# Layjins/Spider

Measured on AMD Instinct MI355X. Metric: multimodal responses/sec (text->text+image), higher is better.
Workload: dtype bf16

## Files before the change

### include/spider_hip.h

```cpp
#ifndef SPIDER_HIP_H
#define SPIDER_HIP_H
#define SPIDER_ABI_VERSION 4

#ifdef __cplusplus
extern "C" {
#endif

int spider_abi_version(void);
const char* spider_target_arch(void);
const char* spider_last_error(void);


int spider_embed_bf16(const void* table, const int* ids, void* out, int rows, int H, int V, void* stream);

int spider_rmsnorm_bf16(const void* x, const void* res, const void* w, void* y, void* res_out, int rows, int H,
                        float eps, void* stream);

int spider_gemv_bf16(const void* W, const void* x, void* out, const void* bias, const void* res, const void* norm_w,
                     float eps, int B, int N, int K, void* stream);

int spider_gemv_swiglu_bf16(const void* W_gate_up, const void* x, void* out, const void* norm_w, float eps, int B,
                            int I, int K, void* stream);

int spider_lm_head_nparts(int V);
// ... 22 lines not shown
int spider_sample_partial_bf16(const void* logits, const void* seen, const void* ban, const float* penalty, const int* min_new,
                               const int* eos_ids, const int* n_eos, const int* n_hist, const int* top_k, float* ws_val,
                               int* ws_tok, int rows, int V, int nslice, void* stream);
int spider_sample_select_f32(const float* ws_val, const int* ws_tok, const float* temperature, const float* top_p, const int* top_k,
                             const void* seed, const int* row0, const int* n_hist, int* next_ids, int* cand_tok, float* cand_p,
                             int* n_keep, float* u, int rows, int V, int nslice, void* stream);

int spider_rope_kv_append_bf16(const void* qkv, const int* pos, const int* slot, const float* cos_sin, void* q_out,
                               void* k_cache, void* v_cache, int B, int S, int n_q, int n_kv, int d, int T_max,
                               void* stream);
int spider_rope_kv_append_mrope_bf16(const void* qkv, const int* pos3, const int* slot, const float* cos_sin, void* q_out,
                                     void* k_cache, void* v_cache, int B, int S, int n_q, int n_kv, int d, int T_max,
                                     int sec_t, int sec_h, void* stream);

int spider_attn_decode_bf16(const void* q, const void* k_cache, const void* v_cache, const int* kv_beg,
                            const int* kv_end, void* out, void* ws_o, void* ws_ml, int B, int n_q, int n_kv, int d,
                            int T_max, float scale, int nsplit, void* stream);

int spider_attn_decode_fused_bf16(const void* qkv, const int* pos, const float* cos_sin, void* k_cache, void* v_cache,
                                  const int* kv_beg, const int* kv_end, void* out, void* ws_o, void* ws_ml,
                                  int* counters, int B, int n_q, int n_kv, int d, int T_max, float scale, int nsplit,
                                  void* stream);
int spider_set_attn_inline(int on);
int spider_set_gemv_sched(int sched);
int spider_set_ws_inlaunch(int on);

int spider_gemv_fm_bf16(const void* Wfm, const void* x, void* out, const void* bias, const void* res, int B, int N, int K,
                        int fold_rmsnorm, float eps, void* stream);
int spider_gemv_swiglu_fm_bf16(const void* Wfm_gate_up, const void* x, void* out, int B, int I, int K, int fold_rmsnorm, float eps,
                               void* stream);
int spider_lm_head_argmax_fm_bf16(const void* Wfm, const void* x, int* out_ids, void* logits, void* ws_val, void* ws_idx, int B,
                                  int V, int K, int fold_rmsnorm, float eps, void* stream);
int spider_lm_head_argmax_fm_proc_bf16(const void* Wfm, const void* x, int* out_ids, void* logits, void* ws_val, void* ws_idx,
                                       const void* seen, const void* ban, const float* penalty, const int* min_new,
                                       const int* eos_ids, const int* n_eos, const int* n_hist, int B, int V, int K,
                                       int fold_rmsnorm, float eps, void* stream);


int spider_gemm_bf16(const void* A, const void* W, void* C, void* C32, const void* bias, const void* res,
                     const void* rowbias, int rows_per_group, int M, int N, int K, int lda, int ldc, int act,
                     float out_scale, int w_tiled, const float* res32, float* c32d, void* ws, long ws_bytes, void* stream);

int spider_gemm_ln_bf16(const void* A, const void* Wf, void* C, const float* colsum, const float* colbias, const void* res,
                        int M, int N, int K, int ldc, int act, float eps, int w_tiled, void* ws, long ws_bytes, void* stream);

int spider_xattn_fused_bf16(const void* x, const void* mq_fm, const void* mo_fm, const float* colsum, const float* colbias,
// ... 193 lines not shown
```

### spider_amd/csrc/llm_decode.hip

```cpp
#include "common.hpp"
#include "select.hpp"
#include <stdlib.h>

using namespace spider;

__global__ __launch_bounds__(256) void embed_kernel(const bf16_t* __restrict__ table, const int* __restrict__ ids,
                                                    bf16_t* __restrict__ out, int H, int V) {
    const int r = blockIdx.x;
    int id = ids[r];
    id = id < 0 ? 0 : (id >= V ? V - 1 : id);
    const u32x4* src = reinterpret_cast<const u32x4*>(table + (size_t)id * H);
    u32x4* dst = reinterpret_cast<u32x4*>(out + (size_t)r * H);
    for (int i = threadIdx.x; i < H / 8; i += 256) dst[i] = src[i];
}

__global__ __launch_bounds__(256) void rope_rows_kernel(bf16_t* __restrict__ x, const float* __restrict__ cs, long row_stride,
                                                        int rows, int heads, int d) {
    const int half = d >> 1, cpr = half >> 3;
    const long total = (long)rows * heads * cpr;
    for (long idx = (long)blockIdx.x * 256 + threadIdx.x; idx < total; idx += (long)gridDim.x * 256) {
        const int c = (int)(idx % cpr);
        const int h = (int)((idx / cpr) % heads);
        const long r = idx / ((long)cpr * heads);
        bf16_t* p = x + r * row_stride + (long)h * d + c * 8;
// ... 803 lines not shown
            o0 = o0 * a + ovv[u].x * bsc;
            o1 = o1 * a + ovv[u].y * bsc;
            m = mn;
        }
    }
    if (lane == 0) { sm_m[wave] = m; sm_l[wave] = l; }
    sm_o[wave][lane * 2] = o0;
    sm_o[wave][lane * 2 + 1] = o1;
    __syncthreads();
    if (threadIdx.x < D) {
        const int dd = threadIdx.x;
        float mm = fmaxf(fmaxf(sm_m[0], sm_m[1]), fmaxf(sm_m[2], sm_m[3]));
        float ll = 0.f, oo = 0.f;
#pragma unroll
        for (int w = 0; w < 4; ++w) {
            const float a = (sm_m[w] == -INFINITY) ? 0.f : __expf(sm_m[w] - mm);
            ll += sm_l[w] * a;
            oo += sm_o[w][dd] * a;
        }
        out[bh * D + dd] = f32_to_bf16(ll > 0.f ? oo / ll : 0.f);
    }
}

template <int D, int G, int NWV, int UR>
__global__ __launch_bounds__(NWV * 64) void attn_decode_fused_kernel(
    const bf16_t* __restrict__ qkv, const int* __restrict__ pos, const float* __restrict__ cs, bf16_t* __restrict__ kc,
    bf16_t* __restrict__ vc, const int* __restrict__ kv_beg, const int* __restrict__ kv_end, float* __restrict__ part_o,
    float* __restrict__ part_ml, int* __restrict__ cnt, bf16_t* __restrict__ out, int n_kv, int T_max, float scale,
    int nsplit, int inline_combine) {
    static_assert(D == 128, "decode attention is specialised for head_dim 128");
    constexpr int HALF = D / 2;
    const int split = blockIdx.x, hk = blockIdx.y, b = blockIdx.z;
    const int n_q = n_kv * G;
    const int lane = threadIdx.x & 63, wave = threadIdx.x >> 6;
    const int sub = lane >> 4;
    const int dl = (lane & 15) * 8;
    const bool hi_half = dl >= HALF;
    const int dp = hi_half ? dl - HALF : dl + HALF;
    const int beg = kv_beg ? kv_beg[b] : 0, end = kv_end[b];
    const int t_new = end - 1;
    const int len_old = max(t_new - beg, 0);
    const int per = (len_old + nsplit - 1) / nsplit;
    const int t0 = beg + split * per, t1 = min(t_new, t0 + per);

    const bf16_t* kbase = kc + ((size_t)b * n_kv + hk) * (size_t)T_max * D;
    const bf16_t* vbase = vc + ((size_t)b * n_kv + hk) * (size_t)T_max * D;
    constexpr int RSTEP = 4 * NWV;
    auto load_rows = [&](int tb_, u32x4 (&kr)[UR], u32x4 (&vr)[UR]) {
#pragma unroll
        for (int u = 0; u < UR; ++u) {
            const int t = min(tb_ + RSTEP * u, t1 - 1);
            kr[u] = *reinterpret_cast<const u32x4*>(kbase + (size_t)t * D + dl);
            vr[u] = *reinterpret_cast<const u32x4*>(vbase + (size_t)t * D + dl);
        }
    };
    const int tb0 = t0 + wave * 4 + sub;
// ... 6 lines not shown
    {
        const int ci = hi_half ? dl - HALF : dl;
        const f32x4 c0 = *reinterpret_cast<const f32x4*>(c + ci), c1 = *reinterpret_cast<const f32x4*>(c + ci + 4);
        const f32x4 s0 = *reinterpret_cast<const f32x4*>(c + HALF + ci), s1 = *reinterpret_cast<const f32x4*>(c + HALF + ci + 4);
#pragma unroll
        for (int j = 0; j < 4; ++j) { cosv[j] = c0[j]; cosv[4 + j] = c1[j]; sinv[j] = s0[j]; sinv[4 + j] = s1[j]; }
    }
    auto rope8 = [&](const bf16_t* head, float (&o)[8]) {
        const u32x4 a = *reinterpret_cast<const u32x4*>(head + dl), pq = *reinterpret_cast<const u32x4*>(head + dp);
        const uint32_t aw[4] = {a.x, a.y, a.z, a.w}, pw[4] = {pq.x, pq.y, pq.z, pq.w};
#pragma unroll
        for (int j = 0; j < 8; ++j) {
            const float xv = (j & 1) ? bf16hi_to_f32(aw[j >> 1]) : bf16lo_to_f32(aw[j >> 1]);
            const float pv = (j & 1) ? bf16hi_to_f32(pw[j >> 1]) : bf16lo_to_f32(pw[j >> 1]);
            const float t1_ = bf16_to_f32(f32_to_bf16(xv * cosv[j]));
            const float t2_ = bf16_to_f32(f32_to_bf16((hi_half ? pv : -pv) * sinv[j]));
            o[j] = bf16_to_f32(f32_to_bf16(t1_ + t2_));
        }
    };

    float qf[G][8];
#pragma unroll
    for (int g = 0; g < G; ++g) {
        rope8(row + (size_t)(hk * G + g) * D, qf[g]);
#pragma unroll
        for (int j = 0; j < 8; ++j) qf[g][j] *= scale;
    }
    float m[G], l[G], o[G][8];
#pragma unroll
    for (int g = 0; g < G; ++g) {
        m[g] = -INFINITY;
        l[g] = 0.f;
#pragma unroll
        for (int j = 0; j < 8; ++j) o[g][j] = 0.f;
    }
    auto update = [&](const float (&kf)[8], const float (&vf)[8]) {
#pragma unroll
        for (int g = 0; g < G; ++g) {
            float sc = 0.f;
#pragma unroll
            for (int j = 0; j < 8; ++j) sc += qf[g][j] * kf[j];
            sc += __shfl_xor(sc, 1, 64);
            sc += __shfl_xor(sc, 2, 64);
            sc += __shfl_xor(sc, 4, 64);
            sc += __shfl_xor(sc, 8, 64);
            const float mn = fmaxf(m[g], sc);
            const float alpha = __expf(m[g] - mn);
// ... 15 lines not shown
                float kf[8], vf[8];
#pragma unroll
                for (int j = 0; j < 4; ++j) {
                    kf[2 * j] = bf16lo_to_f32(kw[j]); kf[2 * j + 1] = bf16hi_to_f32(kw[j]);
                    vf[2 * j] = bf16lo_to_f32(vw[j]); vf[2 * j + 1] = bf16hi_to_f32(vw[j]);
                }
                update(kf, vf);
            }
            if (more) {
                const int t = min(tb + CHUNK + RSTEP * u, t1 - 1);
                kq[u] = *reinterpret_cast<const u32x4*>(kbase + (size_t)t * D + dl);
                vq[u] = *reinterpret_cast<const u32x4*>(vbase + (size_t)t * D + dl);
            }
        }
    }
    if (split == nsplit - 1 && wave == 0 && sub == 0 && t_new >= beg) {
        float kf[8], vf[8];
        rope8(row + (size_t)(n_q + hk) * D, kf);
        const u32x4 vq = *reinterpret_cast<const u32x4*>(row + (size_t)(n_q + n_kv + hk) * D + dl);
        const uint32_t vw[4] = {vq.x, vq.y, vq.z, vq.w};
#pragma unroll
        for (int j = 0; j < 4; ++j) { vf[2 * j] = bf16lo_to_f32(vw[j]); vf[2 * j + 1] = bf16hi_to_f32(vw[j]); }
        update(kf, vf);
        u32x4 ko;
        ko.x = pack_bf16x2(kf[0], kf[1]); ko.y = pack_bf16x2(kf[2], kf[3]);
        ko.z = pack_bf16x2(kf[4], kf[5]); ko.w = pack_bf16x2(kf[6], kf[7]);
        *reinterpret_cast<u32x4*>(kc + (((size_t)b * n_kv + hk) * T_max + t_new) * D + dl) = ko;
        *reinterpret_cast<u32x4*>(vc + (((size_t)b * n_kv + hk) * T_max + t_new) * D + dl) = vq;
    }

    __shared__ float sm_m[NWV][G], sm_l[NWV][G];
    __shared__ float sm_o[NWV][G][D];
    __shared__ int sm_last;
#pragma unroll
    for (int g = 0; g < G; ++g) {
#pragma unroll
        for (int off = 16; off <= 32; off <<= 1) {
            const float m2 = __shfl_xor(m[g], off, 64);
            const float l2 = __shfl_xor(l[g], off, 64);
            const float mn = fmaxf(m[g], m2);
            const float a1 = (m[g] == -INFINITY) ? 0.f : __expf(m[g] - mn);
            const float a2 = (m2 == -INFINITY) ? 0.f : __expf(m2 - mn);
            l[g] = l[g] * a1 + l2 * a2;
#pragma unroll
            for (int j = 0; j < 8; ++j) {
                const float o2 = __shfl_xor(o[g][j], off, 64);
                o[g][j] = o[g][j] * a1 + o2 * a2;
            }
            m[g] = mn;
        }
        if (lane < 16) {
#pragma unroll
            for (int j = 0; j < 8; ++j) sm_o[wave][g][dl + j] = o[g][j];
            if (lane == 0) { sm_m[wave][g] = m[g]; sm_l[wave][g] = l[g]; }
        }
    }
    __syncthreads();
    if (nsplit > 1 && inline_combine) {
        for (int idx = threadIdx.x; idx < G * (D / 4); idx += NWV * 64) {
            const int g = idx / (D / 4), d4 = (idx % (D / 4)) * 4;
            float mm = -INFINITY;
#pragma unroll
            for (int w = 0; w < NWV; ++w) mm = fmaxf(mm, sm_m[w][g]);
            float ll = 0.f;
            f32x4 oo = {0.f, 0.f, 0.f, 0.f};
#pragma unroll
            for (int w = 0; w < NWV; ++w) {
                const float a = (sm_m[w][g] == -INFINITY) ? 0.f : __expf(sm_m[w][g] - mm);
                ll += sm_l[w][g] * a;
#pragma unroll
                for (int j = 0; j < 4; ++j) oo[j] += sm_o[w][g][d4 + j] * a;
            }
            const size_t pi = ((size_t)b * n_q + hk * G + g) * nsplit + split;
            float* po = part_o + pi * D + d4;
            asm volatile("global_store_dwordx4 %0, %1, off sc1" ::"v"(po), "v"(oo) : "memory");
            if (d4 == 0) {
                const float2 mlv = float2{mm, ll};
                float* pm = part_ml + pi * 2;
                asm volatile("global_store_dwordx2 %0, %1, off sc1" ::"v"(pm), "v"(mlv) : "memory");
            }
        }
// ... 49 lines not shown
                }
            }
            const float inv = lsum > 0.f ? 1.f / lsum : 0.f;
            u32x2 o2;
            o2.x = pack_bf16x2(acc[0] * inv, acc[1] * inv);
            o2.y = pack_bf16x2(acc[2] * inv, acc[3] * inv);
            *reinterpret_cast<u32x2*>(out + bh * D + d4) = o2;
        }
        if (threadIdx.x == 0) __hip_atomic_store(cnt + (size_t)b * n_kv + hk, 0, __ATOMIC_RELAXED, __HIP_MEMORY_SCOPE_AGENT);
        return;
    }
    for (int idx = threadIdx.x; idx < G * D; idx += NWV * 64) {
        const int g = idx / D, dd = idx % D;
        float mm = -INFINITY;
#pragma unroll
        for (int w = 0; w < NWV; ++w) mm = fmaxf(mm, sm_m[w][g]);
        float ll = 0.f, oo = 0.f;
#pragma unroll
        for (int w = 0; w < NWV; ++w) {
            const float a = (sm_m[w][g] == -INFINITY) ? 0.f : __expf(sm_m[w][g] - mm);
            ll += sm_l[w][g] * a;
            oo += sm_o[w][g][dd] * a;
        }
        const int hq = hk * G + g;
        if (nsplit == 1) {
            out[((size_t)b * n_q + hq) * D + dd] = f32_to_bf16(ll > 0.f ? oo / ll : 0.f);
        } else {
            const size_t pi = ((size_t)b * n_q + hq) * nsplit + split;
            part_o[pi * D + dd] = oo;
            if (dd == 0) { part_ml[pi * 2] = mm; part_ml[pi * 2 + 1] = ll; }
        }
    }
}

template <bool GATEUP, int NW>
__global__ __launch_bounds__(NW * 64) void skinny_gemm_kernel(const bf16_t* __restrict__ W, const bf16_t* __restrict__ x,
                                                          bf16_t* __restrict__ out, const bf16_t* __restrict__ bias,
                                                          const bf16_t* __restrict__ res, int B, int N, int K) {
    constexpr int TN = GATEUP ? 2 : 1;
    __shared__ float part[NW][TN][64][4];
    const int lane = threadIdx.x & 63, wave = threadIdx.x >> 6;
    const int r16 = lane & 15, g = lane >> 4;
    const int n0 = blockIdx.x * 16;
    const int nrow = min(n0 + r16, N - 1);
    const bf16_t* wrow[TN];
    wrow[0] = W + (size_t)nrow * K + 16 * g;
    if (GATEUP) wrow[1] = W + (size_t)(N + nrow) * K + 16 * g;
    const bool x_ok = r16 < B;
    const bf16_t* xrow = x + (size_t)(x_ok ? r16 : 0) * K + 16 * g;

    const int nkb = K / 64;
    const int kb0 = (wave * nkb) / NW, kb1 = ((wave + 1) * nkb) / NW;
    f32x4 acc[TN];
// ... 291 lines not shown
    if (B >= mfma_min_b && B <= 16 && K % 64 == 0 && norm_w == nullptr) {
        skinny_gemm_kernel<GU, 8><<<(N + 15) / 16, 512, 0, (hipStream_t)stream>>>((const bf16_t*)W, (const bf16_t*)x, (bf16_t*)out,
                                                                                  (const bf16_t*)bias, (const bf16_t*)res, B, N, K);
        SPIDER_LAUNCH_OK();
        return 0;
    }
    switch (B) {
        case 1: return gemv_dispatch<1, GU>(W, x, out, bias, res, norm_w, eps, N, K, stream);
        case 2: return gemv_dispatch<2, GU>(W, x, out, bias, res, norm_w, eps, N, K, stream);
        case 3: return gemv_dispatch<3, GU>(W, x, out, bias, res, norm_w, eps, N, K, stream);
        case 4: return gemv_dispatch<4, GU>(W, x, out, bias, res, norm_w, eps, N, K, stream);
        case 5: return gemv_dispatch<5, GU>(W, x, out, bias, res, norm_w, eps, N, K, stream);
        case 6: return gemv_dispatch<6, GU>(W, x, out, bias, res, norm_w, eps, N, K, stream);
        case 7: return gemv_dispatch<7, GU>(W, x, out, bias, res, norm_w, eps, N, K, stream);
        case 8: return gemv_dispatch<8, GU>(W, x, out, bias, res, norm_w, eps, N, K, stream);
        default: spider_set_error("gemv: batch must be 1..8 (1..16 when K % 64 == 0 and norm_w == NULL; use spider_gemm_bf16 beyond that)"); return -1;
    }
}


#define SPIDER_ATTN_INLINE_DEFAULT 0
static int g_attn_inline = -1;

extern "C" {

int spider_set_gemv_sched(int sched) {
    const int prev = gemv_sched();
    g_gemv_sched = sched != 0;
    return prev;
}

int spider_set_attn_inline(int on) {
    const int prev = g_attn_inline;
    g_attn_inline = on < 0 ? 0 : (on > 2 ? 2 : on);
    return prev;
}

int spider_embed_bf16(const void* table, const int* ids, void* out, int rows, int H, int V, void* stream) {
    SPIDER_CHECK(rows > 0 && H > 0 && H % 8 == 0 && V > 0, "embed: bad shape (H must be a multiple of 8)");
    embed_kernel<<<rows, 256, 0, (hipStream_t)stream>>>((const bf16_t*)table, ids, (bf16_t*)out, H, V);
    SPIDER_LAUNCH_OK();
    return 0;
}

int spider_rope_rows_bf16(void* x, const float* cos_sin, long row_stride, int rows, int heads, int d, void* stream) {
    SPIDER_CHECK(rows > 0 && heads > 0 && d > 0 && d % 16 == 0, "rope_rows: head_dim must be a multiple of 16");
    SPIDER_CHECK(row_stride % 8 == 0 && row_stride >= (long)heads * d, "rope_rows: row stride must be >= heads*d and keep 16-byte alignment");
    const long total = (long)rows * heads * (d / 16);
    long g = (total + 255) / 256;
    if (g > 8192) g = 8192;
    rope_rows_kernel<<<(int)g, 256, 0, (hipStream_t)stream>>>((bf16_t*)x, cos_sin, row_stride, rows, heads, d);
    SPIDER_LAUNCH_OK();
    return 0;
}

int spider_rmsnorm_bf16(const void* x, const void* res, const void* w, void* y, void* res_out, int rows, int H,
                        float eps, void* stream) {
// ... 259 lines not shown
    const int inline_combine = g_attn_inline;
    static const int wide_env = [] { const char* e = getenv("SPIDER_ATTN_WIDE"); return e ? atoi(e) : -1; }();
    const bool wide = wide_env >= 0 ? wide_env != 0 : (T_max / nsplit >= 96);
    switch (G) {
        case 1: ATTN_FUSED_LAUNCH(1); break;
        case 2: ATTN_FUSED_LAUNCH(2); break;
        case 3: ATTN_FUSED_LAUNCH(3); break;
        case 4: ATTN_FUSED_LAUNCH(4); break;
        case 5: ATTN_FUSED_LAUNCH(5); break;
        case 6: ATTN_FUSED_LAUNCH(6); break;
        case 7: ATTN_FUSED_LAUNCH(7); break;
        case 8: ATTN_FUSED_LAUNCH(8); break;
        default: spider_set_error("attn_decode_fused: GQA group size must be 1 ... 8"); return -1;
    }
    SPIDER_LAUNCH_OK();
    if (nsplit > 1 && !inline_combine) {
        attn_combine_kernel<128><<<B * n_q, 256, 0, (hipStream_t)stream>>>((const float*)ws_o, (const float*)ws_ml,
                                                                          (bf16_t*)out, nsplit);
        SPIDER_LAUNCH_OK();
    }
    return 0;
}

}
```

### spider_amd/lib.py

```python
from __future__ import annotations

import ctypes as C
import os
import threading

import torch

_HERE = os.path.dirname(os.path.abspath(__file__))
LIB_PATH = os.path.join(_HERE, "libspider_hip.so")

_lib = None
_lock = threading.Lock()

_vp, _i, _f, _l = C.c_void_p, C.c_int, C.c_float, C.c_long

SIGNATURES = {
    "spider_abi_version": (_i, []),
    "spider_target_arch": (C.c_char_p, []),
    "spider_last_error": (C.c_char_p, []),
    "spider_embed_bf16": (_i, [_vp, _vp, _vp, _i, _i, _i, _vp]),
    "spider_rmsnorm_bf16": (_i, [_vp, _vp, _vp, _vp, _vp, _i, _i, _f, _vp]),
    "spider_gemv_bf16": (_i, [_vp, _vp, _vp, _vp, _vp, _vp, _f, _i, _i, _i, _vp]),
    "spider_gemv_swiglu_bf16": (_i, [_vp, _vp, _vp, _vp, _f, _i, _i, _i, _vp]),
    "spider_lm_head_nparts": (_i, [_i]),
    "spider_decode_advance_i32": (_i, [_vp] * 7 + [_i, _i, _vp]),
    "spider_lm_head_argmax_bf16": (_i, [_vp, _vp, _vp, _f, _vp, _vp, _vp, _vp, _i, _i, _i, _vp]),
    "spider_lm_head_argmax_proc_bf16": (_i, [_vp, _vp, _vp, _f] + [_vp] * 11 + [_i, _i, _i, _vp]),
    "spider_decode_advance_seen_i32": (_i, [_vp] * 8 + [_i, _i, _i, _vp]),
    "spider_token_bitmap_set_i32": (_i, [_vp, _vp, _i, _i, _i, _vp]),
    "spider_beam_partial_bf16": (_i, [_vp] * 4 + [_i] * 4 + [_vp]),
    "spider_beam_select_f32": (_i, [_vp] * 10 + [_i, _vp, _vp] + [_i] * 5 + [_vp]),
    "spider_kv_row_gather_bf16": (_i, [_vp] * 7 + [_i] * 7 + [_vp]),
    "spider_sample_partial_bf16": (_i, [_vp] * 11 + [_i] * 3 + [_vp]),
    "spider_sample_select_f32": (_i, [_vp] * 13 + [_i] * 3 + [_vp]),
    "spider_gemv_fm_bf16": (_i, [_vp, _vp, _vp, _vp, _vp, _i, _i, _i, _i, _f, _vp]),
    "spider_gemv_swiglu_fm_bf16": (_i, [_vp, _vp, _vp, _i, _i, _i, _i, _f, _vp]),
    "spider_lm_head_argmax_fm_bf16": (_i, [_vp, _vp, _vp, _vp, _vp, _vp, _i, _i, _i, _i, _f, _vp]),
    "spider_lm_head_argmax_fm_proc_bf16": (_i, [_vp] * 13 + [_i, _i, _i, _i, _f, _vp]),
    "spider_rope_kv_append_bf16": (_i, [_vp, _vp, _vp, _vp, _vp, _vp, _vp, _i, _i, _i, _i, _i, _i, _vp]),
    "spider_rope_kv_append_mrope_bf16": (_i, [_vp, _vp, _vp, _vp, _vp, _vp, _vp, _i, _i, _i, _i, _i, _i, _i, _i, _vp]),
    "spider_attn_decode_bf16": (_i, [_vp, _vp, _vp, _vp, _vp, _vp, _vp, _vp, _i, _i, _i, _i, _i, _f, _i, _vp]),
    "spider_attn_decode_fused_bf16": (_i, [_vp] * 11 + [_i, _i, _i, _i, _i, _f, _i, _vp]),
    "spider_set_attn_inline": (_i, [_i]),
    "spider_set_gemv_sched": (_i, [_i]),
    "spider_set_ws_inlaunch": (_i, [_i]),
    "spider_gemm_bf16": (_i, [_vp, _vp, _vp, _vp, _vp, _vp, _vp, _i, _i, _i, _i, _i, _i, _i, _f, _i, _vp, _vp, _vp, _l, _vp]),
    "spider_gemm_ln_bf16": (_i, [_vp, _vp, _vp, _vp, _vp, _vp, _i, _i, _i, _i, _i, _f, _i, _vp, _l, _vp]),
    "spider_xattn_fused_bf16": (_i, [_vp, _vp, _vp, _vp, _vp, _vp, _vp, _i, _i, _i, _i, _i, _f, _vp, _vp, _vp]),
    "spider_conv2d_nhwc_bf16": (_i, [_vp, _vp, _vp, _vp, _vp, _vp, _i, _i, _i, _i, _i, _i, _i, _i, _i, _f, _i, _vp, _vp, _vp, _l, _vp]),
    "spider_conv_nhwc_ex_bf16": (_i, [_vp] * 6 + [_i] * 14 + [_f, _f, _i, _vp, _vp, _vp, _l, _vp]),
    "spider_attn_bf16": (_i, [_vp, _vp, _vp, _vp] + [_l] * 12 + [_i] * 6 + [_f, _i, _i, _vp, _vp, _i, _i, _vp]),
    "spider_story_key_lists_i32": (_i, [_vp, _i, _i, _i, _i, _i, _i, _vp, _vp, _vp]),
    "spider_attn_keylist_bf16": (_i, [_vp, _vp, _vp, _vp] + [_l] * 12 + [_i] * 6 + [_f, _vp, _i, _vp, _i, _vp]),
    "spider_attn_varlen_bf16": (_i, [_vp, _vp, _vp, _vp, _l, _l, _l, _l, _i, _i, _i, _i, _f, _vp, _i, _vp]),
    "spider_rope_rows_bf16": (_i, [_vp, _vp, _l, _i, _i, _i, _vp]),
    "spider_groupnorm_nchunk": (_i, [_i]),
    "spider_groupnorm_nhwc_bf16": (_i, [_vp, _vp, _vp, _vp, _vp, _i, _i, _i, _i, _f, _i, _vp]),
    "spider_groupnorm_cat_nhwc_bf16": (_i, [_vp] * 7 + [_i, _i, _i, _i, _i, _f, _i, _vp]),
    "spider_conv_nhwc_gn_bf16": (_i, [_vp] * 6 + [_i] * 14 + [_f, _f, _i, _vp, _vp, _vp, _l, _vp] + [_vp, _i, _vp]),
    "spider_groupnorm_stats_nhwc_bf16": (_i, [_vp, _vp, _i, _i, _i, _i, _i, _vp]),
    "spider_groupnorm_apply_nhwc_bf16": (_i, [_vp, _vp, _i, _vp, _vp, _vp, _i, _i, _i, _i, _f, _i, _vp]),
    "spider_gemm_gn_in_bf16": (_i, [_vp, _vp, _vp, _vp, _i, _i, _i, _i, _i, _vp, _i, _vp, _vp, _i, _f, _i, _vp, _vp]),
    "spider_layernorm_bf16": (_i, [_vp, _vp, _vp, _vp, _i, _i, _f, _vp]),
    "spider_geglu_bf16": (_i, [_vp, _vp, _i, _i, _vp]),
    "spider_swiglu_bf16": (_i, [_vp, _vp, _i, _i, _vp]),
    "spider_concat_channels_bf16": (_i, [_vp, _vp, _vp, _l, _i, _i, _vp]),
# ... 78 lines not shown
```

### spider_amd/llm.py

```python
from __future__ import annotations

import os
import math
from dataclasses import dataclass
from typing import Callable, List, Optional, Sequence

import torch

from . import ops
from .graphs import capture as capture_graph

BF16 = torch.bfloat16


@dataclass
class LLMConfig:
    hidden: int
    layers: int
    n_q: int
    n_kv: int
    head_dim: int
    inter: int
    vocab: int
    rope_theta: float = 10000.0
# ... 525 lines not shown
            q = torch.empty(B, S, c.n_q, c.head_dim, dtype=BF16, device=self.device)
            ops.rope_kv_append(qkv, pos, slot, self.cos_sin, q, k_cache[l], v_cache[l], B, S, c.n_q, c.n_kv, c.head_dim,
                               mrope_section=sec)
            a = ops.attention_cache(q, k_cache[l], v_cache[l], Lk=S, causal=True, kv_off=0, kv_beg=kv_beg)
            h = ops.gemm(a.view(B * S, -1), lw["w_o"], res=h)
            x = ops.rmsnorm(h, lw["ln2"], c.eps)
            if _FUSE_SWIGLU:
                act = ops.gemm(x, lw["w_gu"], act="swiglu")
            else:
                act = ops.swiglu(ops.gemm(x, lw["w_gu"]))
            h = ops.gemm(act, lw["w_down"], res=h)
            if hidden_out is not None:
                hidden_out.append(h.view(B, S, -1).clone())
        return h

    def _decode_step(self, st: dict):
        c, B = self.cfg, st["B"]
        k_cache, v_cache = st["kv"]
        h = ops.embed(self.embed_w, st["cur_ids"]) if st["embeds_in"] is None else st["embeds_in"]
        hs = st.get("hidden_buf")
        if hs is not None:
            hs[0].copy_(h)
        fm = self.fm_batch and B >= self.FM_MIN_BATCH
        fuse_norm = not fm and B < 5
        for l, lw in enumerate(self.layers):
            if fuse_norm:
                ops.gemv(lw["w_qkv"], h, bias=lw["b_qkv"], norm_w=lw["ln1"], eps=c.eps, out=st["qkv"])
            elif fm:
                ops.gemv_fm(lw["w_qkv_fm"], h, lw["w_qkv"].shape[0], bias=lw["b_qkv"], out=st["qkv"], norm_eps=c.eps)
            else:
                ops.gemv(lw["w_qkv"], ops.rmsnorm(h, lw["ln1"], c.eps, out=st["xn"]), bias=lw["b_qkv"], out=st["qkv"])
            if c.head_dim == 128:
                ops.attn_decode_fused(st["qkv"], st["pos"], self.cos_sin, k_cache[l], v_cache[l], st["kv_end"],
                                      st["kv_beg"], st["attn_cnt"], c.n_q, st["nsplit"], st["attn_ws"], st["attn"])
            else:
                ops.rope_kv_append(st["qkv"], st["pos"], st["slot"], self.cos_sin, st["q"], k_cache[l], v_cache[l],
                                   B, 1, c.n_q, c.n_kv, c.head_dim)
                ops.attn_decode(st["q"], k_cache[l], v_cache[l], st["kv_end"], kv_beg=st["kv_beg"],
                                nsplit=st["nsplit"], ws=st["attn_ws"], out=st["attn"])
            if fm:
                h1 = ops.gemv_fm(lw["w_o_fm"], st["attn"], c.hidden, res=h, out=st["h1"])
                ops.gemv_swiglu_fm(lw["w_gu_fm"], h1, out=st["act"], norm_eps=c.eps)
                h = ops.gemv_fm(lw["w_down_fm"], st["act"], c.hidden, res=h1, out=st["h2"][l & 1])
            else:
                h1 = ops.gemv(lw["w_o"], st["attn"], res=h, out=st["h1"])
                if fuse_norm:
                    ops.gemv_swiglu(lw["w_gu"], h1, norm_w=lw["ln2"], eps=c.eps, out=st["act"])
                else:
                    ops.gemv_swiglu(lw["w_gu"], ops.rmsnorm(h1, lw["ln2"], c.eps, out=st["xn"]), out=st["act"])
                h = ops.gemv(lw["w_down"], st["act"], res=h1, out=st["h2"][l & 1])
            if hs is not None:
                hs[l + 1].copy_(h)
        if st.get("beam") is not None:
            bm = st["beam"]
            if fm:
                ops.lm_head_argmax_fm(self.lm_head_fm, h, c.vocab, out_ids=bm["lm_ids"], ws=st["lm_ws"], logits=st["logits"],
                                      norm_eps=c.eps)
            else:
                ops.lm_head_argmax(self.lm_head, h, norm_w=self.norm, eps=c.eps, out_ids=bm["lm_ids"], ws=st["lm_ws"],
                                   logits=st["logits"])
            self._beam_step(st)
            return
        proc = st.get("proc")
        if st.get("sample") is not None:
            if fm:
                ops.lm_head_argmax_fm(self.lm_head_fm, h, c.vocab, out_ids=st["sample"]["lm_ids"], ws=st["lm_ws"], logits=st["logits"],
                                      norm_eps=c.eps)
            else:
# ... 14 lines not shown
                               logits=st.get("logits"))
        if hs is not None:
            ops.rmsnorm(h, self.norm, c.eps, out=hs[c.layers])
        if proc is not None:
            ops.decode_advance_seen(st["next_ids"], st["cur_ids"], st["pos"], st["slot"], st["kv_end"], st["seen"], c.vocab,
                                    st["hist"], st["n_hist"])
        else:
            ops.decode_advance(st["next_ids"], st["cur_ids"], st["pos"], st["slot"], st["kv_end"], st["hist"], st["n_hist"])

    def _sample_step(self, st: dict):
        ops.sample_partial(st["logits"], st["sample"], st.get("proc"))
        ops.sample_select(st["sample"], st["n_hist"], st["next_ids"], self.cfg.vocab)

    def _beam_step(self, st: dict, reorder: bool = True):
        bm, c = st["beam"], self.cfg
        ops.beam_partial(st["logits"], bm["C"], bm["ws"])
        ops.beam_select(bm["ws"], bm["run"], bm["eos_ids"], bm["n_eos"], st["n_hist"], bm["trace"], bm["src_beam"], st["next_ids"],
                        c.vocab, bm["C"])
        if reorder:
            ops.kv_row_gather(st["kv"][0], st["kv"][1], bm["kv_tmp"][0], bm["kv_tmp"][1], bm["src_beam"], st["kv_beg"], st["kv_end"],
                              bm["K"])
            ops.decode_advance(st["next_ids"], st["cur_ids"], st["pos"], st["slot"], st["kv_end"], st["hist"], st["n_hist"])

    _PROC_BUFS = ("seen", "ban", "penalty", "min_new", "eos_ids", "n_eos")

    def _make_state(self, B: int, want_hidden: bool, want_logits: bool, cache_set: int = 0, processed: bool = False,
                    beam: Optional[tuple] = None, sample: bool = False) -> dict:
        c, dv = self.cfg, self.device
        nq_d = c.n_q * c.head_dim
        nsplit = max(1, min(64, 256 // max(1, B * c.n_kv)))
        if os.environ.get("SPIDER_ATTN_NSPLIT"):
            nsplit = int(os.environ["SPIDER_ATTN_NSPLIT"])
        i32 = lambda *s: torch.zeros(*s, dtype=torch.int32, device=dv)
        bf = lambda *s: torch.empty(*s, dtype=BF16, device=dv)
        npart = ops.lm_head_nparts(c.vocab)
        st = dict(B=B, nsplit=nsplit, cur_ids=i32(B), next_ids=i32(B), pos=i32(B), slot=i32(B), kv_end=i32(B), kv_beg=i32(B),
                  qkv=bf(B, (c.n_q + 2 * c.n_kv) * c.head_dim), q=bf(B, c.n_q, c.head_dim), attn=bf(B, nq_d),
                  h1=bf(B, c.hidden), h2=[bf(B, c.hidden), bf(B, c.hidden)], act=bf(B, c.inter), xn=bf(B, c.hidden),
                  attn_ws=(torch.empty(B * c.n_q * nsplit * c.head_dim, dtype=torch.float32, device=dv),
                           torch.empty(B * c.n_q * nsplit * 2, dtype=torch.float32, device=dv)),
                  lm_ws=(torch.empty(B * npart, dtype=torch.float32, device=dv), i32(B * npart)),
                  attn_cnt=i32(B * c.n_kv), embeds_in=None, hist=i32(B, self.max_len), n_hist=i32(B), kv=self._kv(cache_set))
        if want_hidden:
            st["hidden_buf"] = bf(c.layers + 1, B, c.hidden)
        if want_logits:
            st["logits"] = bf(B, c.vocab)
        if processed:
            W = ops.bitmap_words(c.vocab)
            st.update(seen=i32(B, W), ban=i32(B, W), penalty=torch.ones(1, dtype=torch.float32, device=dv), min_new=i32(1),
                      eos_ids=i32(MAX_EOS_IDS), n_eos=i32(1))
            st["proc"] = {k: st[k] for k in self._PROC_BUFS + ("n_hist",)}
        if sample:
            st["sample"] = dict(ops.sample_state(B, c.vocab, dv), lm_ids=i32(B))
        if beam is not None:
            K, C = beam
            nb = B // K
            if cache_set not in self._beam_kv_tmp:
                self._beam_kv_tmp[cache_set] = (torch.zeros_like(self.k_cache), torch.zeros_like(self.v_cache))
            st["beam"] = dict(K=K, C=C, run=torch.zeros(nb, K, dtype=torch.float32, device=dv), src_beam=i32(nb, K), lm_ids=i32(B),
                              eos_ids=i32(MAX_EOS_IDS), n_eos=i32(1), ws=ops.beam_workspace(B, c.vocab, C, dv),
                              trace=(torch.zeros(self.max_len, nb, C, dtype=torch.float32, device=dv), i32(self.max_len, nb, C),
                                     i32(self.max_len, nb, C)),
                              kv_tmp=self._beam_kv_tmp[cache_set])
# ... 340 lines not shown
```

### spider_amd/ops.py

```python
from __future__ import annotations

import ctypes as C
import math
from typing import Optional

import torch

from . import lib as _lib

BF16 = torch.bfloat16
ACT = {None: 0, "none": 0, "silu": 1, "gelu": 2, "quick_gelu": 3, "geglu": 4, "leaky_relu": 5, "relu": 6, "tanh": 7, "swiglu": 8,
       "geglu_exact": 9}
GLU_ACTS = ("geglu", "swiglu", "geglu_exact")


def _stream() -> int:
    return torch.cuda.current_stream().cuda_stream


_WS = {}
WS_BYTES = 64 << 20
WS_TAIL = 4096


# ... 480 lines not shown
    if out is None:
        out = torch.empty(B, n_q * d, dtype=BF16, device=q.device)
    if nsplit > 1 and ws is None:
        ws = (torch.empty(B * n_q * nsplit * d, dtype=torch.float32, device=q.device),
              torch.empty(B * n_q * nsplit * 2, dtype=torch.float32, device=q.device))
    _lib.call("spider_attn_decode_bf16", _p(q), _p(k_cache), _p(v_cache), _p(kv_beg), _p(kv_end), _p(out),
              _p(ws[0]) if ws else None, _p(ws[1]) if ws else None, B, n_q, n_kv, d, T_max, float(scale), nsplit, _stream())
    return out


def attn_decode_fused(qkv, pos, cos_sin, k_cache, v_cache, kv_end, kv_beg, counters, n_q, nsplit, ws, out, scale=None):
    _chk(qkv, BF16, "qkv"); _chk(pos, torch.int32, "pos"); _chk(cos_sin, torch.float32, "cos_sin")
    _chk(k_cache, BF16, "k_cache"); _chk(v_cache, BF16, "v_cache"); _chk(kv_end, torch.int32, "kv_end")
    _chk(counters, torch.int32, "counters"); _chk(out, BF16, "out")
    B = kv_end.numel()
    n_kv, T_max, d = k_cache.shape[1], k_cache.shape[2], k_cache.shape[3]
    assert qkv.numel() == B * (n_q + 2 * n_kv) * d and counters.numel() >= B * n_kv and cos_sin.shape[1] == d
    if scale is None:
        scale = 1.0 / math.sqrt(d)
    _lib.call("spider_attn_decode_fused_bf16", _p(qkv), _p(pos), _p(cos_sin), _p(k_cache), _p(v_cache), _p(kv_beg), _p(kv_end),
              _p(out), _p(ws[0]) if ws else None, _p(ws[1]) if ws else None, _p(counters), B, n_q, n_kv, d, T_max,
              float(scale), nsplit, _stream())
    return out


def gemm(A, W, bias=None, res=None, rowbias=None, rows_per_group=0, act=None, out_scale=1.0, out=None, out_f32=False,
         res32=None, want32=False):
    dt, sfx = _h16(A)
    _chk(A, dt, "A"); _chk(W, dt, "W")
    N, K = W.shape
    assert A.shape[-1] == K, f"gemm: A[..., {A.shape[-1]}] vs W[{N},{K}]"
    M = A.numel() // K
    n_out = N // 2 if act in GLU_ACTS else N
    if out is None:
        out = torch.empty(*A.shape[:-1], n_out, dtype=torch.float32 if out_f32 else dt, device=A.device)
    c16, c32 = (None, out) if out.dtype == torch.float32 else (out, None)
    wt = _tiled(W, M)
    o32 = torch.empty(out.shape, dtype=torch.float32, device=A.device) if want32 else None
    if res32 is not None:
        _chk(res32, torch.float32, "res32")
    _lib.call(f"spider_gemm_{sfx}", _p(A), _p(W if wt is None else wt), _p(c16), _p(c32), _p(bias), _p(res), _p(rowbias), rows_per_group,
              M, N, K, K, n_out, ACT[act], float(out_scale), int(wt is not None), _p(res32), _p(o32), _p(_workspace(A.device)), WS_BYTES,
              _stream())
    return (out, o32) if want32 else out


# ... 742 lines not shown
```

Measured before the change: 2.006.

## Fold split-KV attention combine into o_proj GEMV with query-head split decode

For batch-1 decode, attention now runs as a query-head-split kernel (one query head per block, split along KV), and it writes only the per-split partial outputs plus their max and sum. The o_proj GEMV then merges those partials itself while its weight loads are in flight, and computes the output projection from the combined vector held in shared memory. This removes the separate combine step and the bf16 attention-output round trip, and it spreads decode attention over more blocks to fill the GPU. In exchange, every o_proj block repeats the partial merge, and the path applies only to small shapes (n_q*d <= 4096, within a workspace budget).

```diff
diff --git a/include/spider_hip.h b/include/spider_hip.h
--- a/include/spider_hip.h
+++ b/include/spider_hip.h
@@ -68,6 +68,14 @@
                                   int* counters, int B, int n_q, int n_kv, int d, int T_max, float scale, int nsplit,
                                   void* stream);
 int spider_set_attn_inline(int on);
+
+int spider_attn_combine_bf16(const void* ws_o, const void* ws_ml, void* out, int rows, int d, int nsplit, void* stream);
+int spider_attn_decode_qsplit_bf16(const void* qkv, const int* pos, const float* cos_sin, void* k_cache, void* v_cache,
+                                   const int* kv_beg, const int* kv_end, void* out, void* ws_o, void* ws_ml, int B, int n_q,
+                                   int n_kv, int d, int T_max, float scale, int nsplit, void* stream);
+int spider_gemv_attn_partials_bf16(const void* W, const void* ws_o, const void* ws_ml, void* out, const void* bias, const void* res,
+                                   int N, int n_q, int d, int nsplit, void* stream);
+int spider_set_attn_fold(int on);
 int spider_set_gemv_sched(int sched);
 int spider_set_ws_inlaunch(int on);
 
diff --git a/spider_amd/csrc/llm_decode.hip b/spider_amd/csrc/llm_decode.hip
--- a/spider_amd/csrc/llm_decode.hip
+++ b/spider_amd/csrc/llm_decode.hip
@@ -849,7 +849,7 @@
     }
 }
 
-template <int D, int G, int NWV, int UR>
+template <int D, int G, int NWV, int UR, bool QS = false>
 __global__ __launch_bounds__(NWV * 64) void attn_decode_fused_kernel(
     const bf16_t* __restrict__ qkv, const int* __restrict__ pos, const float* __restrict__ cs, bf16_t* __restrict__ kc,
     bf16_t* __restrict__ vc, const int* __restrict__ kv_beg, const int* __restrict__ kv_end, float* __restrict__ part_o,
@@ -857,8 +857,10 @@
     int nsplit, int inline_combine) {
     static_assert(D == 128, "decode attention is specialised for head_dim 128");
     constexpr int HALF = D / 2;
-    const int split = blockIdx.x, hk = blockIdx.y, b = blockIdx.z;
-    const int n_q = n_kv * G;
+    static_assert(!QS || G == 1, "the query-split form serves one query head per block");
+    const int split = QS ? blockIdx.x % nsplit : blockIdx.x, hk = QS ? blockIdx.x / nsplit : blockIdx.y, b = blockIdx.z;
+    const int n_q = QS ? n_kv * gridDim.y : n_kv * G;
+    const int hq0 = QS ? hk * gridDim.y + blockIdx.y : hk * G;
     const int lane = threadIdx.x & 63, wave = threadIdx.x >> 6;
     const int sub = lane >> 4;
     const int dl = (lane & 15) * 8;
@@ -911,7 +913,7 @@
     float qf[G][8];
 #pragma unroll
     for (int g = 0; g < G; ++g) {
-        rope8(row + (size_t)(hk * G + g) * D, qf[g]);
+        rope8(row + (size_t)(hq0 + g) * D, qf[g]);
 #pragma unroll
         for (int j = 0; j < 8; ++j) qf[g][j] *= scale;
     }
@@ -973,11 +975,13 @@
 #pragma unroll
         for (int j = 0; j < 4; ++j) { vf[2 * j] = bf16lo_to_f32(vw[j]); vf[2 * j + 1] = bf16hi_to_f32(vw[j]); }
         update(kf, vf);
-        u32x4 ko;
-        ko.x = pack_bf16x2(kf[0], kf[1]); ko.y = pack_bf16x2(kf[2], kf[3]);
-        ko.z = pack_bf16x2(kf[4], kf[5]); ko.w = pack_bf16x2(kf[6], kf[7]);
-        *reinterpret_cast<u32x4*>(kc + (((size_t)b * n_kv + hk) * T_max + t_new) * D + dl) = ko;
-        *reinterpret_cast<u32x4*>(vc + (((size_t)b * n_kv + hk) * T_max + t_new) * D + dl) = vq;
+        if (!QS || blockIdx.y == 0) {
+            u32x4 ko;
+            ko.x = pack_bf16x2(kf[0], kf[1]); ko.y = pack_bf16x2(kf[2], kf[3]);
+            ko.z = pack_bf16x2(kf[4], kf[5]); ko.w = pack_bf16x2(kf[6], kf[7]);
+            *reinterpret_cast<u32x4*>(kc + (((size_t)b * n_kv + hk) * T_max + t_new) * D + dl) = ko;
+            *reinterpret_cast<u32x4*>(vc + (((size_t)b * n_kv + hk) * T_max + t_new) * D + dl) = vq;
+        }
     }
 
     __shared__ float sm_m[NWV][G], sm_l[NWV][G];
@@ -1007,7 +1011,7 @@
         }
     }
     __syncthreads();
-    if (nsplit > 1 && inline_combine) {
+    if (!QS && nsplit > 1 && inline_combine) {
         for (int idx = threadIdx.x; idx < G * (D / 4); idx += NWV * 64) {
             const int g = idx / (D / 4), d4 = (idx % (D / 4)) * 4;
             float mm = -INFINITY;
@@ -1103,13 +1107,127 @@
             ll += sm_l[w][g] * a;
             oo += sm_o[w][g][dd] * a;
         }
-        const int hq = hk * G + g;
+        const int hq = hq0 + g;
         if (nsplit == 1) {
             out[((size_t)b * n_q + hq) * D + dd] = f32_to_bf16(ll > 0.f ? oo / ll : 0.f);
         } else {
             const size_t pi = ((size_t)b * n_q + hq) * nsplit + split;
             part_o[pi * D + dd] = oo;
             if (dd == 0) { part_ml[pi * 2] = mm; part_ml[pi * 2 + 1] = ll; }
+        }
+    }
+}
+
+template <int R, int SB>
+__global__ __launch_bounds__(512) void gemv_attn_partials_kernel(const bf16_t* __restrict__ W, const float* __restrict__ part_o,
+                                                                 const float* __restrict__ part_ml, bf16_t* __restrict__ out,
+                                                                 const bf16_t* __restrict__ bias, const bf16_t* __restrict__ res,
+                                                                 int N, int K, int nsplit) {
+    constexpr int D = 128, NWB = 8, H = 8;
+    extern __shared__ __attribute__((aligned(16))) char smem[];
+    bf16_t* xs = reinterpret_cast<bf16_t*>(smem);
+    const int lane = threadIdx.x & 63, wave = __builtin_amdgcn_readfirstlane(threadIdx.x >> 6);
+    const int nv = K / 8;
+    const int i = min((int)threadIdx.x, nv - 1);
+    const size_t p0 = (size_t)(i >> 4) * nsplit;
+    const int d8 = (i & 15) * 8;
+    float2 ml[SB];
+    f32x4 po[SB][2];
+    auto issue_p = [&](int s0) {
+#pragma unroll
+        for (int u = 0; u < SB; ++u) ml[u] = *reinterpret_cast<const float2*>(part_ml + (p0 + min(s0 + u, nsplit - 1)) * 2);
+#pragma unroll
+        for (int u = 0; u < SB; ++u) {
+            const float* o = part_o + (p0 + min(s0 + u, nsplit - 1)) * D + d8;
+            po[u][0] = *reinterpret_cast<const f32x4*>(o);
+            po[u][1] = *reinterpret_cast<const f32x4*>(o + 4);
+        }
+    };
+    issue_p(0);
+
+    const int col0 = (blockIdx.x * NWB + wave) * R;
+    const bf16_t* wrow[R];
+#pragma unroll
+    for (int r = 0; r < R; ++r) {
+        const int n = col0 + r;
+        wrow[r] = W + (size_t)(n < N ? n : N - 1) * K;
+    }
+    u32x4 w0[H][R];
+#pragma unroll
+    for (int u = 0; u < H; ++u) {
+        const int k = lane * 8 + u * 512;
+#pragma unroll
+        for (int r = 0; r < R; ++r)
+            w0[u][r] = __builtin_nontemporal_load(reinterpret_cast<const u32x4*>(wrow[r] + (unsigned)(k < K ? k : K - 8)));
+    }
+
+    float m = -INFINITY, l = 0.f, o[8];
+#pragma unroll
+    for (int j = 0; j < 8; ++j) o[j] = 0.f;
+    auto merge_p = [&](int s0) {
+#pragma unroll
+        for (int u = 0; u < SB; ++u) {
+            if (s0 + u < nsplit) {
+                const float ms = ml[u].x, ls = ml[u].y;
+                const float mn = fmaxf(m, ms);
+                const float a = (m == -INFINITY) ? 0.f : __expf(m - mn);
+                const float bsc = (ms == -INFINITY) ? 0.f : __expf(ms - mn);
+                l = l * a + ls * bsc;
+#pragma unroll
+                for (int j = 0; j < 4; ++j) {
+                    o[j] = o[j] * a + po[u][0][j] * bsc;
+                    o[4 + j] = o[4 + j] * a + po[u][1][j] * bsc;
+                }
+                m = mn;
+            }
+        }
+    };
+    merge_p(0);
+    for (int s0 = SB; s0 < nsplit; s0 += SB) {
+        issue_p(s0);
+        merge_p(s0);
+    }
+    {
+        float a[8];
+#pragma unroll
+        for (int j = 0; j < 8; ++j) a[j] = l > 0.f ? o[j] / l : 0.f;
+        u32x4 av;
+        av.x = pack_bf16x2(a[0], a[1]); av.y = pack_bf16x2(a[2], a[3]);
+        av.z = pack_bf16x2(a[4], a[5]); av.w = pack_bf16x2(a[6], a[7]);
+        reinterpret_cast<u32x4*>(xs)[i] = av;
+    }
+    __syncthreads();
+
+    if (col0 >= N) return;
+    float acc[R];
+#pragma unroll
+    for (int r = 0; r < R; ++r) acc[r] = 0.f;
+#pragma unroll
+    for (int u = 0; u < H; ++u) {
+        const int k = lane * 8 + u * 512;
+        if (k < K) {
+            const u32x4 xq = *reinterpret_cast<const u32x4*>(xs + k);
+            const uint32_t xw[4] = {xq.x, xq.y, xq.z, xq.w};
+#pragma unroll
+            for (int r = 0; r < R; ++r) {
+                const uint32_t ww[4] = {w0[u][r].x, w0[u][r].y, w0[u][r].z, w0[u][r].w};
+#pragma unroll
+                for (int j = 0; j < 4; ++j) acc[r] = dot2_bf16(ww[j], xw[j], acc[r]);
+            }
+        }
+    }
+#pragma unroll
+    for (int r = 0; r < R; ++r) acc[r] = wave_sum(acc[r]);
+    if (lane == 0) {
+#pragma unroll
+        for (int r = 0; r < R; ++r) {
+            const int n = col0 + r;
+            if (n < N) {
+                float v = acc[r];
+                if (bias) v += bf16_to_f32(bias[n]);
+                if (res) v = bf16_to_f32(f32_to_bf16(v)) + bf16_to_f32(res[n]);
+                out[n] = f32_to_bf16(v);
+            }
         }
     }
 }
@@ -1447,6 +1565,13 @@
 #define SPIDER_ATTN_INLINE_DEFAULT 0
 static int g_attn_inline = -1;
 
+#define SPIDER_ATTN_FOLD_DEFAULT 1
+static int g_attn_fold = -1;
+static int attn_fold() {
+    if (g_attn_fold < 0) { const char* e = getenv("SPIDER_ATTN_FOLD"); g_attn_fold = e ? (atoi(e) != 0) : SPIDER_ATTN_FOLD_DEFAULT; }
+    return g_attn_fold;
+}
+
 extern "C" {
 
 int spider_set_gemv_sched(int sched) {
@@ -1458,6 +1583,12 @@
 int spider_set_attn_inline(int on) {
     const int prev = g_attn_inline;
     g_attn_inline = on < 0 ? 0 : (on > 2 ? 2 : on);
+    return prev;
+}
+
+int spider_set_attn_fold(int on) {
+    const int prev = attn_fold();
+    if (on >= 0) g_attn_fold = on != 0;
     return prev;
 }
 
@@ -1763,4 +1894,47 @@
     return 0;
 }
 
-}
+
+int spider_attn_combine_bf16(const void* ws_o, const void* ws_ml, void* out, int rows, int d, int nsplit, void* stream) {
+    SPIDER_CHECK(d == 128, "attn_combine: head_dim must be 128");
+    SPIDER_CHECK(rows > 0 && nsplit >= 1 && ws_o && ws_ml && out, "attn_combine: bad shape");
+    attn_combine_kernel<128><<<rows, 256, 0, (hipStream_t)stream>>>((const float*)ws_o, (const float*)ws_ml, (bf16_t*)out, nsplit);
+    SPIDER_LAUNCH_OK();
+    return 0;
+}
+
+#define ATTN_QSPLIT_ARGS                                                                                        \
+    (const bf16_t*)qkv, pos, cos_sin, (bf16_t*)k_cache, (bf16_t*)v_cache, kv_beg, kv_end, (float*)ws_o, (float*)ws_ml, nullptr, \
+        (bf16_t*)out, n_kv, T_max, scale, nsplit, 0
+
+int spider_attn_decode_qsplit_bf16(const void* qkv, const int* pos, const float* cos_sin, void* k_cache, void* v_cache,
+                                   const int* kv_beg, const int* kv_end, void* out, void* ws_o, void* ws_ml, int B, int n_q,
+                                   int n_kv, int d, int T_max, float scale, int nsplit, void* stream) {
+    SPIDER_CHECK(d == 128, "attn_decode_qsplit: head_dim must be 128");
+    SPIDER_CHECK(B > 0 && n_kv > 0 && n_q % n_kv == 0 && nsplit >= 1 && T_max > 0, "attn_decode_qsplit: bad shape");
+    SPIDER_CHECK(nsplit == 1 ? out != nullptr : (ws_o && ws_ml), "attn_decode_qsplit: out (nsplit == 1) or workspace (nsplit > 1) required");
+    SPIDER_CHECK(n_q / n_kv <= 65535 && B <= 65535, "attn_decode_qsplit: grid too large");
+    dim3 grid(n_kv * nsplit, n_q / n_kv, B);
+    static const int wide_env = [] { const char* e = getenv("SPIDER_ATTN_WIDE"); return e ? atoi(e) : -1; }();
+    const bool wide = wide_env >= 0 ? wide_env != 0 : (T_max / nsplit >= 96);
+    if (wide) attn_decode_fused_kernel<128, 1, 8, 8, true><<<grid, 512, 0, (hipStream_t)stream>>>(ATTN_QSPLIT_ARGS);
+    else attn_decode_fused_kernel<128, 1, 4, 4, true><<<grid, 256, 0, (hipStream_t)stream>>>(ATTN_QSPLIT_ARGS);
+    SPIDER_LAUNCH_OK();
+    return 0;
+}
+
+int spider_gemv_attn_partials_bf16(const void* W, const void* ws_o, const void* ws_ml, void* out, const void* bias, const void* res,
+                                   int N, int n_q, int d, int nsplit, void* stream) {
+    SPIDER_CHECK(d == 128, "gemv_attn_partials: head_dim must be 128");
+    SPIDER_CHECK(N > 0 && n_q > 0 && n_q * d <= 4096 && nsplit >= 1, "gemv_attn_partials: bad shape (n_q * d <= 4096)");
+    const int K = n_q * d;
+    static const int r_env = [] { const char* e = getenv("SPIDER_ATTN_FOLD_R"); return e ? atoi(e) : 2; }();
+#define FOLD_ARGS (const bf16_t*)W, (const float*)ws_o, (const float*)ws_ml, (bf16_t*)out, (const bf16_t*)bias, (const bf16_t*)res, N, K, nsplit
+    if (r_env == 1) gemv_attn_partials_kernel<1, 8><<<(N + 7) / 8, 512, (size_t)K * 2, (hipStream_t)stream>>>(FOLD_ARGS);
+    else gemv_attn_partials_kernel<2, 8><<<(N + 15) / 16, 512, (size_t)K * 2, (hipStream_t)stream>>>(FOLD_ARGS);
+#undef FOLD_ARGS
+    SPIDER_LAUNCH_OK();
+    return 0;
+}
+
+}
diff --git a/spider_amd/lib.py b/spider_amd/lib.py
--- a/spider_amd/lib.py
+++ b/spider_amd/lib.py
@@ -42,6 +42,10 @@
     "spider_attn_decode_bf16": (_i, [_vp, _vp, _vp, _vp, _vp, _vp, _vp, _vp, _i, _i, _i, _i, _i, _f, _i, _vp]),
     "spider_attn_decode_fused_bf16": (_i, [_vp] * 11 + [_i, _i, _i, _i, _i, _f, _i, _vp]),
     "spider_set_attn_inline": (_i, [_i]),
+    "spider_attn_combine_bf16": (_i, [_vp, _vp, _vp, _i, _i, _i, _vp]),
+    "spider_attn_decode_qsplit_bf16": (_i, [_vp] * 10 + [_i, _i, _i, _i, _i, _f, _i, _vp]),
+    "spider_gemv_attn_partials_bf16": (_i, [_vp] * 6 + [_i, _i, _i, _i, _vp]),
+    "spider_set_attn_fold": (_i, [_i]),
     "spider_set_gemv_sched": (_i, [_i]),
     "spider_set_ws_inlaunch": (_i, [_i]),
     "spider_gemm_bf16": (_i, [_vp, _vp, _vp, _vp, _vp, _vp, _vp, _i, _i, _i, _i, _i, _i, _i, _f, _i, _vp, _vp, _vp, _l, _vp]),
diff --git a/spider_amd/llm.py b/spider_amd/llm.py
--- a/spider_amd/llm.py
+++ b/spider_amd/llm.py
@@ -571,6 +571,7 @@
         if hs is not None:
             hs[0].copy_(h)
         fm = self.fm_batch and B >= self.FM_MIN_BATCH
+        fold = B == 1 and not fm and st.get("beam") is None and st["nsplit_q"] > 1 and ops.attn_fold() != 0
         fuse_norm = not fm and B < 5
         for l, lw in enumerate(self.layers):
             if fuse_norm:
@@ -579,7 +580,10 @@
                 ops.gemv_fm(lw["w_qkv_fm"], h, lw["w_qkv"].shape[0], bias=lw["b_qkv"], out=st["qkv"], norm_eps=c.eps)
             else:
                 ops.gemv(lw["w_qkv"], ops.rmsnorm(h, lw["ln1"], c.eps, out=st["xn"]), bias=lw["b_qkv"], out=st["qkv"])
-            if c.head_dim == 128:
+            if fold:
+                ops.attn_decode_qsplit(st["qkv"], st["pos"], self.cos_sin, k_cache[l], v_cache[l], st["kv_end"], st["kv_beg"],
+                                       c.n_q, st["nsplit_q"], st["attn_ws"])
+            elif c.head_dim == 128:
                 ops.attn_decode_fused(st["qkv"], st["pos"], self.cos_sin, k_cache[l], v_cache[l], st["kv_end"],
                                       st["kv_beg"], st["attn_cnt"], c.n_q, st["nsplit"], st["attn_ws"], st["attn"])
             else:
@@ -592,7 +596,10 @@
                 ops.gemv_swiglu_fm(lw["w_gu_fm"], h1, out=st["act"], norm_eps=c.eps)
                 h = ops.gemv_fm(lw["w_down_fm"], st["act"], c.hidden, res=h1, out=st["h2"][l & 1])
             else:
-                h1 = ops.gemv(lw["w_o"], st["attn"], res=h, out=st["h1"])
+                if fold:
+                    h1 = ops.gemv_attn_partials(lw["w_o"], st["attn_ws"], c.n_q, st["nsplit_q"], res=h, out=st["h1"])
+                else:
+                    h1 = ops.gemv(lw["w_o"], st["attn"], res=h, out=st["h1"])
                 if fuse_norm:
                     ops.gemv_swiglu(lw["w_gu"], h1, norm_w=lw["ln2"], eps=c.eps, out=st["act"])
                 else:
@@ -653,6 +660,8 @@
                               bm["K"])
             ops.decode_advance(st["next_ids"], st["cur_ids"], st["pos"], st["slot"], st["kv_end"], st["hist"], st["n_hist"])
 
+    ATTN_FOLD_BUDGET = 128 << 10
+
     _PROC_BUFS = ("seen", "ban", "penalty", "min_new", "eos_ids", "n_eos")
 
     def _make_state(self, B: int, want_hidden: bool, want_logits: bool, cache_set: int = 0, processed: bool = False,
@@ -662,14 +671,24 @@
         nsplit = max(1, min(64, 256 // max(1, B * c.n_kv)))
         if os.environ.get("SPIDER_ATTN_NSPLIT"):
             nsplit = int(os.environ["SPIDER_ATTN_NSPLIT"])
+        nsplit_q = 0
+        if B == 1 and c.head_dim == 128 and nq_d <= 4096:
+            nsplit_q = max(2, min(8, 256 // c.n_q))
+            if (c.n_kv * nsplit_q) % 8 and nsplit_q > 2 and (c.n_kv * (nsplit_q - 1)) % 8 == 0:
+                nsplit_q -= 1
+            if os.environ.get("SPIDER_ATTN_NSPLIT_Q"):
+                nsplit_q = int(os.environ["SPIDER_ATTN_NSPLIT_Q"])
+            if c.n_q * nsplit_q * 4 * c.head_dim > self.ATTN_FOLD_BUDGET:
+                nsplit_q = 0
         i32 = lambda *s: torch.zeros(*s, dtype=torch.int32, device=dv)
         bf = lambda *s: torch.empty(*s, dtype=BF16, device=dv)
         npart = ops.lm_head_nparts(c.vocab)
-        st = dict(B=B, nsplit=nsplit, cur_ids=i32(B), next_ids=i32(B), pos=i32(B), slot=i32(B), kv_end=i32(B), kv_beg=i32(B),
+        nws = max(nsplit, nsplit_q)
+        st = dict(B=B, nsplit=nsplit, nsplit_q=nsplit_q, cur_ids=i32(B), next_ids=i32(B), pos=i32(B), slot=i32(B), kv_end=i32(B), kv_beg=i32(B),
                   qkv=bf(B, (c.n_q + 2 * c.n_kv) * c.head_dim), q=bf(B, c.n_q, c.head_dim), attn=bf(B, nq_d),
                   h1=bf(B, c.hidden), h2=[bf(B, c.hidden), bf(B, c.hidden)], act=bf(B, c.inter), xn=bf(B, c.hidden),
-                  attn_ws=(torch.empty(B * c.n_q * nsplit * c.head_dim, dtype=torch.float32, device=dv),
-                           torch.empty(B * c.n_q * nsplit * 2, dtype=torch.float32, device=dv)),
+                  attn_ws=(torch.empty(B * c.n_q * nws * c.head_dim, dtype=torch.float32, device=dv),
+                           torch.empty(B * c.n_q * nws * 2, dtype=torch.float32, device=dv)),
                   lm_ws=(torch.empty(B * npart, dtype=torch.float32, device=dv), i32(B * npart)),
                   attn_cnt=i32(B * c.n_kv), embeds_in=None, hist=i32(B, self.max_len), n_hist=i32(B), kv=self._kv(cache_set))
         if want_hidden:
diff --git a/spider_amd/ops.py b/spider_amd/ops.py
--- a/spider_amd/ops.py
+++ b/spider_amd/ops.py
@@ -526,6 +526,51 @@
               _p(out), _p(ws[0]) if ws else None, _p(ws[1]) if ws else None, _p(counters), B, n_q, n_kv, d, T_max,
               float(scale), nsplit, _stream())
     return out
+
+
+def attn_decode_qsplit(qkv, pos, cos_sin, k_cache, v_cache, kv_end, kv_beg, n_q, nsplit, ws, out=None, scale=None):
+    _chk(qkv, BF16, "qkv"); _chk(pos, torch.int32, "pos"); _chk(cos_sin, torch.float32, "cos_sin")
+    _chk(k_cache, BF16, "k_cache"); _chk(v_cache, BF16, "v_cache"); _chk(kv_end, torch.int32, "kv_end")
+    B = kv_end.numel()
+    n_kv, T_max, d = k_cache.shape[1], k_cache.shape[2], k_cache.shape[3]
+    assert qkv.numel() == B * (n_q + 2 * n_kv) * d and cos_sin.shape[1] == d
+    if nsplit > 1:
+        _chk(ws[0], torch.float32, "ws[0]"); _chk(ws[1], torch.float32, "ws[1]")
+        assert ws[0].numel() >= B * n_q * nsplit * d and ws[1].numel() >= B * n_q * nsplit * 2
+    else:
+        _chk(out, BF16, "out")
+        assert out.numel() == B * n_q * d
+    if scale is None:
+        scale = 1.0 / math.sqrt(d)
+    _lib.call("spider_attn_decode_qsplit_bf16", _p(qkv), _p(pos), _p(cos_sin), _p(k_cache), _p(v_cache), _p(kv_beg), _p(kv_end),
+              _p(out), _p(ws[0]) if ws else None, _p(ws[1]) if ws else None, B, n_q, n_kv, d, T_max, float(scale), nsplit, _stream())
+    return out
+
+
+def attn_combine(ws, rows, nsplit, out=None, d=128):
+    _chk(ws[0], torch.float32, "ws[0]"); _chk(ws[1], torch.float32, "ws[1]")
+    assert ws[0].numel() >= rows * nsplit * d and ws[1].numel() >= rows * nsplit * 2
+    if out is None:
+        out = torch.empty(rows, d, dtype=BF16, device=ws[0].device)
+    _chk(out, BF16, "out")
+    assert out.numel() == rows * d
+    _lib.call("spider_attn_combine_bf16", _p(ws[0]), _p(ws[1]), _p(out), rows, d, nsplit, _stream())
+    return out
+
+
+def gemv_attn_partials(W, ws, n_q, nsplit, bias=None, res=None, out=None, d=128):
+    _chk(W, BF16, "W"); _chk(ws[0], torch.float32, "ws[0]"); _chk(ws[1], torch.float32, "ws[1]")
+    N, K = W.shape
+    assert K == n_q * d and ws[0].numel() >= n_q * nsplit * d and ws[1].numel() >= n_q * nsplit * 2
+    if out is None:
+        out = torch.empty(1, N, dtype=BF16, device=W.device)
+    assert out.numel() == N and (res is None or res.numel() == N) and (bias is None or bias.numel() == N)
+    _lib.call("spider_gemv_attn_partials_bf16", _p(W), _p(ws[0]), _p(ws[1]), _p(out), _p(bias), _p(res), N, n_q, d, nsplit, _stream())
+    return out
+
+
+def attn_fold(on: int = -1) -> int:
+    return _lib.load().spider_set_attn_fold(int(on))
 
 
 def gemm(A, W, bias=None, res=None, rowbias=None, rows_per_group=0, act=None, out_scale=1.0, out=None, out_f32=False,
```

Result: no change. 2.026, median of 6 (+1.0%).
